# mike-gimelfarb/bboptpy

Hardware: AMD Instinct MI355X
Metric: candidate-evals/sec (higher is better)
Workload: dtype f64; 1 GPU; ActiveCMAES n=128 np=4096 rosenbrock, 256 independent populations per GPU in lockstep; populations_per_gpu=256, n=128, np=4096, objective=rosenbrock

## Files before the change

bboptpy_amd/csrc/bbo_cma.hip:

```cpp
#include "bbo_cma_kernels.hpp"
#include "bbo_sep_kernels.hpp"
#include "bbo_chol_kernels.hpp"
#include "bbo_eig_mw.hpp"

#include <algorithm>
#include <atomic>
#include <cmath>
#include <cstdlib>
#include <limits>

namespace bbo {

namespace {

enum { K_SAMPLE = 0, K_RANK, K_WHITEN, K_GRAM, K_PATHS, K_COV, K_EIGEN, K_POST, K_STOP, K_COUNT };
static const char *const K_NAMES[K_COUNT] = { "bbo:cma_sample_eval", "bbo:cma_rank", "bbo:cma_whiten", "bbo:cma_gram", "bbo:cma_paths", "bbo:cma_cov", "bbo:cma_eigen", "bbo:cma_post", "bbo:cma_history_stop" };

int pick_maxt(int ld)
{
    const int per_wave = ((ld >> 4) + 3) / 4;
    if (per_wave <= 1) return 1;
    if (per_wave <= 2) return 2;
    if (per_wave <= 4) return 4;
    return 8;
// ... 537 lines not shown
        if (c.ld == 128 && (long) c.npop * c.mu_pad >= 256 * 128) {
            const int rw = rows_per_workgroup((long) c.npop * c.mu_pad, 2048);
            add(UK_WHITEN128, K_WHITEN, (c.mu_pad + rw - 1) / rw, c.npop, 1, 512, (size_t) (128 * 128 + 128) * sizeof(double),
                    rw);
        } else
            add(UK_WHITEN, K_WHITEN, c.mu_pad / 16, c.npop, 1, 256, (size_t) (16 * (c.ld + 2) + 64) * sizeof(double),
                    pick_maxt(c.ld));
    }
    if (c.ld != 128)
        add(UK_GRAM, K_GRAM, c.splits, (LT + 4 * GRAM_TPW - 1) / (4 * GRAM_TPW), c.npop, 256, gram_lds_bytes(c.ld, c.rps),
                gram_ldy(c.ld));
    else if (d_.dbg & DBG_GRAM128_LDS)
        add(UK_GRAM128, K_GRAM, c.splits, c.npop, 1, 256, (size_t) (2 * G128_CH * G128_LDY + 4 * G128_CH) * sizeof(double));
    else
        add(UK_GRAM128S, K_GRAM, c.splits, c.npop, 1, 256);
    if (c.lazy_isc && c.n >= 64 && !(d_.dbg & DBG_PATHS_LAZY256))
        add(UK_PATHS_LAZY1K, K_PATHS, c.npop, 1, 1, 1024);
    else
        add(c.lazy_isc ? UK_PATHS_LAZY : UK_PATHS, K_PATHS, c.npop, 1, 1, 256);
    if (with_cov) add(UK_COV, K_COV, (c.n * (c.n + 1) / 2 + 255) / 256, c.npop, 1, 256);
    return r;
}

static auto whiten_kernel(int maxt) -> void (*)(CmaDev, CmaConst)
{
    switch (maxt) {
    case 1: return cma_whiten<1>;
    case 2: return cma_whiten<2>;
    case 4: return cma_whiten<4>;
    default: return cma_whiten<8>;
    }
}

// ... 10 lines not shown
        };
        timed(s.slot, [&] {
            switch (s.k) {
            case UK_CHOL_PATHS: go(chol_paths, 0); break;
            case UK_CHOL_CPRIME: go(chol_cprime, 0); break;
            case UK_CHOL_FACTOR: go(chol_factor, 0, s.arg); break;
            case UK_SEP_MOMENTS: go(sep_moments, 0); break;
            case UK_SEP_PATHS: go(sep_paths, 0); break;
            case UK_WHITEN128: go(cma_whiten128, 132 * 1024, s.arg); break;
            case UK_WHITEN: go(whiten_kernel(s.arg), s.arg == 8 ? 80 * 1024 : 0); break;
            case UK_GRAM128S: go(cma_gram128s, 0); break;
            case UK_GRAM128: go(cma_gram128, 80 * 1024); break;
            case UK_GRAM: go(cma_gram, (int) GRAM_LDS_MAX, s.arg); break;
            case UK_PATHS: go(cma_paths, 0); break;
            case UK_PATHS_LAZY: go(cma_paths_lazy, 0); break;
            case UK_PATHS_LAZY1K: go(cma_paths_lazy1k, 0); break;
            case UK_COV: go(cma_cov, 0); break;
            }
        });
    }
    last_update_ = r;
}

int CmaEngine::next_mw_xcd()
{
    static std::atomic<int> counter { 0 };
    return counter.fetch_add(1) & 7;
}

EigRoute CmaEngine::eig_route(bool spread_ok, bool fuse_ok) const
{
// ... 5 lines not shown
    const EigPlan pl_lds = eig_plan(c.n, c.ld);
    r.split = pl_lds.use_lds && pl_lds.threads == 512 && pl_lds.dc && c.npop <= split_maxp_
            && !(dbg & (DBG_QL | DBG_DC_NO_MERGES | DBG_DC_NO_LEAVES | DBG_TRED_L2 | DBG_EIG_ONE_WG));
    const EigPlan pl = r.split ? eig_plan_split(c.n, c.ld) : pl_lds;
    spread_ok = spread_ok && !mw_disabled_;
    const bool fixed_shape = c.n == 128 && c.ld == 128 && !d_.stamps
            && !(dbg & (DBG_EIG_IN_KERNEL | DBG_EIG_GENERIC128));
    bool big_spread = false, wy4_packs = false, fcols_closed = false;
    if (c.n <= 16 && c.n >= 2 && c.ld == 16 && !(dbg & DBG_NO_EIGEN_SMALL))
        add(EK_EIGEN_SMALL);
    else if (pl.threads < 512)
        add(pl.threads == 128 ? EK_EIGEN_128 : EK_EIGEN_256);
    else if (fixed_shape && c.npop > split_maxp_ && c.lazy_isc) {
        r.fixed = true;
        r.forms_c = fuse_ok && !(dbg & DBG_COV_UNFUSED);
        add(r.forms_c ? EK_EIGEN_FX128 : EK_EIGEN_FX128U);
    } else if (pl.use_lds)
        add(EK_EIGEN);
    else if (pl.hybrid && !(dbg & (DBG_QL | DBG_TRED_L2 | DBG_EIG_ONE_WG))) {
        if (r.split) {
            r.fixed = fixed_shape;
            add(r.fixed ? EK_EIGEN_R1_FX128 : EK_EIGEN_R1);
        } else if (spread_ok && !(dbg & DBG_TRED_ONE_WG)) {
            r.mw_workgroups = (long) c.npop * MW_G;
            const int istop = (dbg & DBG_TRED_ALL_SPREAD) ? 1 : 128;
            add(EK_TRED_MW, istop);
            if (istop > 1) add(EK_TRED_TAIL);
        } else
            add(EK_EIGEN_G1);
        add(EK_EIG_HALVES);
// ... 29 lines not shown
            add(EK_EIG_WY4_512);
        else if ((dbg & DBG_QL) || !pl.hybrid)
            add(EK_EIG_GEMM, 1);
        else if ((long) c.npop * ((c.n + 15) / 16) <= 256 && !(dbg & DBG_WY_PER_WAVE)) {
            wy4_packs = c.lazy_isc != 0;
            add(EK_EIG_WY4, wy4_packs ? (fcols_closed ? 2 : 1) : 0);
        } else
            add(EK_EIG_WY);
    }
    const bool packed_by_eigen = c.lazy_isc && pl.dc && pl.reg_path && !(dbg & DBG_QL);
    r.post = r.step[0].k != EK_EIGEN_SMALL && !packed_by_eigen && !wy4_packs;
    if (r.post) add(c.ld <= 128 ? EK_POST_MFMA : EK_POST);
    return r;
}

void CmaEngine::launch_eigen(EigRoute r)
{
    const CmaConst &c = c_;
    if (r.mw_workgroups && !mw_reserve(r.mw_workgroups)) r = eig_route(false, r.forms_c);
    last_route_ = r;
    if (c.variant >= 2) return;
    const EigPlan pl_lds = eig_plan(c.n, c.ld), pl = r.split ? eig_plan_split(c.n, c.ld) : pl_lds;
    const EigFxArgs fa { d_.C, d_.B, d_.D, d_.BDp, d_.eig_work, d_.scal, c.eigenfreq, c.honor_stop,
            c.splits, c.variant, d_.gram_part, d_.pc, c.cc, c.c1, c.cmu, c.cneg, c.alphaold };
    auto per_matrix = [&](auto kernel, int threads, const EigPlan &p, auto... args) {
        allow_lds((const void*) kernel, 160 * 1024 - 768);
        hipLaunchKernelGGL(kernel, dim3(c.npop), dim3(threads), p.lds_bytes, stream_, args...);
    };
    auto per_columns = [&](auto kernel, int w, int threads, auto... args) {
        hipLaunchKernelGGL(kernel, dim3((c.n + w - 1) / w, c.npop), dim3(threads), 0, stream_, d_, c_, args...);
    };
    timer_.begin(stream_, K_EIGEN);
    for (int i = 0; i < r.count; i++) {
        if (i == r.timed) {
            timer_.end(stream_);
            BBO_HIP(hipGetLastError());
        }
        const int arg = r.step[i].arg;
        switch (r.step[i].k) {
// ... 125 lines not shown
void CmaEngine::generation(bool honor_stop)
{
    if (small_fused_ok()) {
        launch_small(1, honor_stop);
        return;
    }
    small_fused_ = false;
    c_.honor_stop = honor_stop ? 1 : 0;
    launch_sample_eval();
    if (obj_.needs_host()) host_evaluate();
    else if (obj_.is_program()) program_evaluate();
    launch_rank();
    const EigRoute route = eig_route(true, true);
    launch_update(!route.forms_c);
    launch_eigen(route);
    launch_history_stop();
}

void CmaEngine::phase(int which)
{
    BBO_REQUIRE(inited_, "phase before init");
    BBO_HIP(hipSetDevice(params_.device));
    c_.honor_stop = 0;
    d_.mw_fault = mw_fault_from_env();
    switch (which) {
    case BBO_PHASE_SAMPLE_EVALUATE:
        launch_sample_eval();
        if (obj_.needs_host()) host_evaluate();
        else if (obj_.is_program()) program_evaluate();
        break;
    case BBO_PHASE_RANK: launch_rank(); break;
// ... 240 lines not shown
    if (k == "eig_stage") return o.one(s.eig_stage);
    if (k == "eig_mw_fail") return o.one(s.eig_mw_fail);
    if (k == "chol_repairs") {
        if (c.variant != 3) throw Error(BBO_ERR_KEY, "'chol_repairs' belongs to CholeskyCMAES");
        int r = 0;
        chol_repairs_.download(&r, 1, p);
        return o.one(r);
    }
    if (c.variant == 3 && k == "chol_tri") return o.one(chol_tri_ ? 1 : 0);
    if (c.variant == 3 && k == "stol") return o.one(c.stol);
    if (c.variant == 3 && k == "ranked") return o.one(c.ranked);
    if (k == "eig_mw_off") return o.one(mw_disabled_ ? 1 : 0);
    if (k == "eig_split_maxp") return o.one(split_maxp_);
    if (k == "eig_fixed128") return o.one(last_route_.fixed ? 1 : 0);
    if (k == "cov_fused") return o.one(last_route_.forms_c ? 1 : 0);
    if (k == "eig_route") {
        double ids[sizeof(last_route_.step) / sizeof(last_route_.step[0])];
        for (int i = 0; i < last_route_.count; i++) ids[i] = last_route_.step[i].k;
        return o.copy(ids, last_route_.count);
    }
    if (k == "rank_route") return o.one(last_rank_);
    if (k == "sample_route") return o.one(last_sample_.k);
    if (k == "sample_lean") return o.one(last_sample_.full);
    if (k == "sample_transposed") return o.one(last_sample_.transposed);
    if (k == "sample128_rowlayout") return o.one(sample128_rowlayout_ ? 1 : 0);
    if (k == "update_route") {
        double ids[sizeof(last_update_.step) / sizeof(last_update_.step[0])];
        for (int i = 0; i < last_update_.count; i++) ids[i] = last_update_.step[i].k;
        return o.copy(ids, last_update_.count);
    }
// ... 135 lines not shown
        chol_tri_ = in[0] != 0.;
        return 1;
    }
    if (k == "sample_wide_max") {
        sample_wide_max_tiles_ = (long) in[0];
        return 1;
    }
    if (k == "sample128_rowlayout") {
        sample128_rowlayout_ = in[0] != 0.;
        return 1;
    }
    if (k == "sample128_min") {
        sample128_min_rows_ = (long) in[0];
        return 1;
    }
    if (k == "eig_split_maxp") {
        split_maxp_ = (int) in[0];
        return 1;
    }
    if (k == "stop_off") {
        c_.stop_off = (int) in[0];
        return 1;
    }
    if (k == "ftarget") {
        c_.ftarget = in[0];
        return 1;
    }
    if (k == "eig_stamps") {
        if (stamps_.count != 48) stamps_.alloc(48);
        BBO_HIP(hipStreamSynchronize(stream_));
// ... 53 lines not shown
```

bboptpy_amd/csrc/bbo_cma.hpp:

```cpp
#pragma once

#include "bbo_engine.hpp"

namespace bbo {

struct CmaScal {
    double sigma;
    double fbest, fworst;
    double pslen;
    double ybw[4];
    int ibw[4];
    int it, fev;
    int flag;
    int stop;
    int hsig;
    int eigenlastev, eigen_done;
    int hist_head, hist_len;
    int basis_ok;
    int eig_stage;
    int eig_mw_fail;
};

struct CmaConst {
    int n, ld;
// ... 96 lines not shown
    EK_POST, EK_POST_MFMA
};

struct EigRoute {
    struct Step {
        EigKernel k;
        int arg;
    };
    Step step[12];
    int count;
    int timed;
    bool split;
    bool post;
    bool fixed;
    bool forms_c;
    long mw_workgroups;
};

enum SampleKernel : int {
    SK_NONE = -1,
    SK_SEP_16 = 0, SK_SEP_64_512, SK_SEP_64_512_LEAN, SK_SEP_SUM, SK_SEP_SUM4, SK_SEP_64,
    SK_EVAL128, SK_EVAL128_TRI, SK_TILE8, SK_TILE8_TRI,
    SK_EVAL64_1_8, SK_EVAL64_1, SK_EVAL64_2,
    SK_TILE16, SK_EVAL_4, SK_EVAL_8
};

struct SampleRoute {
    SampleKernel k;
    int gx, gy, block;
    size_t lds;
// ... 7 lines not shown
    UK_CHOL_PATHS = 0, UK_CHOL_CPRIME, UK_CHOL_FACTOR, UK_SEP_MOMENTS, UK_SEP_PATHS,
    UK_WHITEN128, UK_WHITEN, UK_GRAM128S, UK_GRAM128, UK_GRAM,
    UK_PATHS, UK_PATHS_LAZY, UK_PATHS_LAZY1K, UK_COV
};

struct UpdateRoute {
    struct Step {
        UpdateKernel k;
        int slot;
        int gx, gy, gz, block;
        size_t lds;
        int arg;
    };
    Step step[4];
    int count;
};

class CmaEngine: public Engine<CmaScal> {
public:
    static constexpr const char *HANDLE_NAME = "not a CMA-ES handle";
    explicit CmaEngine(const bbo_params &p);
    ~CmaEngine() override;

    void init(int n, const double *lower, const double *upper, const double *guess,
            const ObjectiveSpec &obj) override;
    void solution(int population, double *x_out, int *n_evals, int *converged) override;
    void optimize(int n, const double *lower, const double *upper, const double *guess,
            const ObjectiveSpec &obj, double *x_out, int *n_evals, int *converged) override;
    int get(const std::string &key, int population, double *out, int cap) override;
    int set(const std::string &key, int population, const double *in, int count) override;
    int dimension() const override { return c_.n; }
// ... 41 lines not shown

    CmaConst c_ {};
    CmaDev d_ {};
    bool keep_bc_ = false;
    bool basis_maybe_stale_ = false;
    DevBuf<double> mw_buf_;
    unsigned long long mw_launch_ = 0;
    bool mw_disabled_ = false;
    int mw_xcd_ = next_mw_xcd();
    static int next_mw_xcd();
    long sample_wide_max_tiles_ = 512;
    long sample128_min_rows_ = 256 * 128;
    bool chol_tri_ = true;
    bool sample128_rowlayout_ = false;
    int split_maxp_ = 32;
    EigRoute last_route_ {};
    SampleRoute last_sample_ { SK_NONE };
    UpdateRoute last_update_ {};
    bool small_fused_ = false;
    int last_rank_ = -1;
    bool rank_wrote_norms_ = false;
    int last_n_ = -1;

    DevBuf<double> zn2_, csep_, A_;
    DevBuf<double> X_, f_, xmean_, xold_, pc_, ps_, C_, B_, D_, isc_, BDp_, ISp_, S_,
            gram_part_, mean_part_, hist_best_, hist_kth_, eig_work_, weights_, zinject_, zrecord_;
    DevBuf<double> coef_tab_;
    DevBuf<int> rank_, order_, chol_repairs_, coef_stamp_;
    void coef_tab_forget();
    DevBuf<long long> stamps_;
// ... 10 lines not shown
```

bboptpy_amd/csrc/bbo_cma_kernels.hpp:

```cpp
#pragma once

#include "bbo_cma.hpp"
#include "bbo_objectives.hpp"
#include "bbo_rng.hpp"
#include "bbo_eig.hpp"
#include "bbo_rank.hpp"

namespace bbo {

typedef double d4_t __attribute__((ext_vector_type(4)));

#define BBO_INF (__builtin_huge_val())

__device__ inline void cma_draw_quad(const CmaDev &d, const CmaConst &c, int p, int row, int q,
        int gen, uint32_t sw, const double2 *tab, double (&z)[4])
{
    const int j0 = cma_quad_col0(q);
    z[0] = z[1] = z[2] = z[3] = 0.;
    if (row < c.lambda && j0 < c.n) {
        if (d.zinject) {
            const double *zi = d.zinject + ((size_t) p * c.lambda + row) * c.n;
#pragma unroll
            for (int i = 0; i < 4; i++)
                if (j0 + 4 * i < c.n) z[i] = zi[j0 + 4 * i];
// ... 1278 lines not shown
__global__ __launch_bounds__(256, 2) void cma_gram128s(CmaDev d, CmaConst c)
{
    const int p = blockIdx.y, s = blockIdx.x;
    if (pop_frozen(c, d.scal + p)) return;
    __shared__ double coef[4][2 * 2 * G128_CH];
    const int lane = threadIdx.x & 63, wave = threadIdx.x >> 6;
    const bool use_tab = d.coef_tab && !(d.dbg & DBG_GRAM_LOOKUP) && d.coef_stamp[p] == d.scal[p].it + 1;
    switch (wave) {
    case 0: gram128_stream<0>(d, c, p, s, coef[0], lane, use_tab); break;
    case 1: gram128_stream<1>(d, c, p, s, coef[1], lane, use_tab); break;
    case 2: gram128_stream<2>(d, c, p, s, coef[2], lane, use_tab); break;
    default: gram128_stream<3>(d, c, p, s, coef[3], lane, use_tab); break;
    }
}

template<bool LAZY = false, int T = 256>
__device__ __forceinline__ void paths_body(const CmaDev &d, const CmaConst &c, int p)
{
    CmaScal *sc = d.scal + p;
    if (pop_frozen(c, sc)) return;
    __shared__ double dm[512];
    __shared__ double red[T / 64];
    const int tid = threadIdx.x, ld = c.ld;
    double *xmean = d.xmean + (size_t) p * ld, *xold = d.xold + (size_t) p * ld;
    double *ps = d.ps + (size_t) p * ld, *pc = d.pc + (size_t) p * ld;
    const double sigma = sc->sigma;

    for (int j = tid; j < ld; j += T) {
        double sum = 0.;
        {
            const double *mp = d.mean_part + (size_t) p * c.splits * ld + j;
            int s = 0;
            for (; s + 8 <= c.splits; s += 8) {
                double x[8];
#pragma unroll
// ... 3 lines not shown
                for (int u = 0; u < 8; u++) sum += x[u];
            }
            for (; s < c.splits; s++) sum += mp[(size_t) s * ld];
        }
        const double xo = xmean[j];
        sum = xo + sigma * sum;
        double xn = 0.;
        if (j < c.n) {
            xn = c.variant == 1 ? xo * (1. - c.cm) + sum * c.cm : sum;
            if (c.bound) xn = fmax(d.lower[j], fmin(xn, d.upper[j]));
        }
        xold[j] = xo;
        xmean[j] = xn;
        dm[j] = xn - xo;
    }
    __syncthreads();

    const double csc = sqrt(c.cs * (2. - c.cs) * c.mueff);
    const double den = c.variant == 1 ? c.cm * sigma : sigma;
    const double *isc = d.isc + (size_t) p * ld * ld;
    double ssq = 0.;
    if (LAZY && sc->basis_ok) {
        constexpr int HN = T / 128;
        constexpr int RS = T / 16, NU = 128 / RS;
        __shared__ double sv[256], cv[256], part[HN - 1][128];
        const double *B = d.B + (size_t) p * ld * ld, *D = d.D + (size_t) p * ld;
        for (int jb = 0; jb < c.n; jb += 128) {
            const int j = jb + (tid & 127), h = tid >> 7;
            double t0 = 0., t1 = 0., t2 = 0., t3 = 0.;
            if (j < c.n) {
                int i = h;
                for (; i + 7 * HN < c.n; i += 8 * HN) {
                    double b[8];
#pragma unroll
                    for (int u = 0; u < 8; u++) b[u] = B[(size_t) (i + HN * u) * ld + j];
                    t0 += b[0] * dm[i] + b[4] * dm[i + 4 * HN];
                    t1 += b[1] * dm[i + HN] + b[5] * dm[i + 5 * HN];
                    t2 += b[2] * dm[i + 2 * HN] + b[6] * dm[i + 6 * HN];
                    t3 += b[3] * dm[i + 3 * HN] + b[7] * dm[i + 7 * HN];
                }
                for (; i < c.n; i += HN) t0 += B[(size_t) i * ld + j] * dm[i];
            }
            const double t = (t0 + t1) + (t2 + t3);
            if (h > 0) part[h - 1][tid & 127] = t;
            __syncthreads();
            if (h == 0) {
                double tt = t;
#pragma unroll
                for (int q = 0; q < HN - 1; q++) tt += part[q][tid & 127];
                sv[j] = j < c.n ? tt / D[j] : 0.;
            }
            __syncthreads();
        }
        for (int ib = 0; ib < c.n; ib += 128) {
            const int g = tid & 15, r = ib + (tid >> 4);
            double a[NU];
#pragma unroll
            for (int u = 0; u < NU; u++) {
                const int i = r + RS * u;
                double tot = 0.;
                for (int kb = 0; kb < c.n; kb += 128) {
                    double x[8];
#pragma unroll
                    for (int k = 0; k < 8; k++) {
                        const int j = kb + g + 16 * k;
                        x[k] = (i < c.n && j < c.n) ? B[(size_t) i * ld + j] * sv[j] : 0.;
                    }
                    const double part8 = ((x[0] + x[1]) + (x[2] + x[3])) + ((x[4] + x[5]) + (x[6] + x[7]));
                    tot = kb == 0 ? part8 : tot + part8;
                }
                a[u] = tot;
            }
#pragma unroll
            for (int u = 0; u < NU; u++) {
                const double v = group_sum<16>(a[u]);
                if (g == 0 && r + RS * u < c.n) cv[r + RS * u] = v;
            }
        }
        __syncthreads();
        for (int i = tid; i < ld; i += T) {
            const double v = i < c.n ? (1. - c.cs) * ps[i] + csc * cv[i] / den : 0.;
            ps[i] = v;
            ssq += v * v;
        }
    } else {
        for (int i = tid; i < ld; i += T) {
            double v = 0.;
            if (i < c.n) {
                double acc = 0.;
                for (int j = 0; j < c.n; j++) acc += isc[(size_t) j * ld + i] * dm[j];
                v = (1. - c.cs) * ps[i] + csc * acc / den;
            }
            ps[i] = v;
// ... 26 lines not shown
        if (sc->it >= c.hlen && sc->fworst - sc->fbest == 0.) sg *= exp(0.2 + c.cs / c.damps);
        sc->sigma = sg;
        sc->hsig = hsig;
        sc->pslen = pslen;
    }
}

__global__ __launch_bounds__(256) void cma_paths(CmaDev d, CmaConst c)
{
    paths_body<false>(d, c, blockIdx.x);
}
__global__ __launch_bounds__(256) void cma_paths_lazy(CmaDev d, CmaConst c)
{
    paths_body<true>(d, c, blockIdx.x);
}
__global__ __launch_bounds__(1024) void cma_paths_lazy1k(CmaDev d, CmaConst c)
{
    paths_body<true, 1024>(d, c, blockIdx.x);
}

__device__ __forceinline__ void cov_body(const CmaDev &d, const CmaConst &c, int p, int bx)
{
    const CmaScal *sc = d.scal + p;
    if (pop_frozen(c, sc)) return;
    const int q = bx * 256 + threadIdx.x;
    const int total = c.n * (c.n + 1) / 2;
    if (q >= total) return;
    int i, j;
    tri_tile(q, i, j);
    const int ld = c.ld;
    double *C = d.C + (size_t) p * ld * ld;
    const double *pc = d.pc + (size_t) p * ld;
    const double cij = C[(size_t) i * ld + j];
// ... 200 lines not shown
    }
    if (mode == 2) {
        for (int q = q0 + tid; q < q1; q += 256) {
            const int t4 = q >> 6, l = q & 63;
            const int nt = t4 / KS, ks = t4 - nt * KS;
            const int i = nt * 16 + (l & 15), j = 4 * ks + (l >> 4);
            ISp[q] = (i < n && j < n) ? isc[(size_t) i * ld + j] : 0.;
        }
    }
}

__device__ __forceinline__ void history_stop_body(const CmaDev &d, const CmaConst &c, int p, int lane)
{
    CmaScal *sc = d.scal + p;
    if (pop_frozen(c, sc)) return;
    const int ld = c.ld, n = c.n;
    double *hb = d.hist_best + (size_t) p * c.hlen, *hk = d.hist_kth + (size_t) p * c.hlen;
    const double *f = d.f + (size_t) p * c.lambda_pad;
    const int *order = d.order + (size_t) p * c.lambda_pad;
    int it = sc->it;
    int head = sc->hist_head, len = sc->hist_len;
    double fbest = sc->fbest, fworst = sc->fworst;

    if (it < c.mit) {
        head = (head + 1) % c.hlen;
        if (lane == 0) {
            hb[head] = f[order[0]];
            hk[head] = f[order[c.ik]];
        }
        if (len < c.hlen) len++;
        wave_sync();
        if (len == c.hlen) {
            double lo = BBO_INF, hi = -BBO_INF;
            for (int k = lane; k < c.hlen; k += 64) {
                lo = fmin(lo, hb[k]);
                hi = fmax(hi, hb[k]);
            }
#pragma unroll
            for (int off = 32; off > 0; off >>= 1) {
                lo = fmin(lo, __shfl_xor(lo, off, 64));
                hi = fmax(hi, __shfl_xor(hi, off, 64));
            }
            fbest = lo;
            fworst = hi;
        }
    }
    it++;
    wave_sync();

    const double sigma = sc->sigma;
    const double *pc = d.pc + (size_t) p * ld, *xm = d.xmean + (size_t) p * ld;
    const double *C = d.C + (size_t) p * ld * ld, *B = d.B + (size_t) p * ld * ld;
    const double *D = d.D + (size_t) p * ld;
    int flag = 0;
    const int off = c.stop_off;
    if (it >= c.mit) {
        flag = 1;
    } else if (f[order[0]] <= c.ftarget) {
        flag = 10;
    } else if (!(off & 4) && it >= c.hlen && fworst - fbest < c.tol) {
        flag = 2;
    } else {
        if (!(off & 8) && len >= n) {
            int eq = 0;
            for (int i = lane; i < n; i += 64) {
                const int idx = (c.hlen + head - i) % c.hlen;
                eq += hb[idx] == hk[idx];
            }
#pragma unroll
            for (int off = 32; off > 0; off >>= 1) eq += __shfl_xor(eq, off, 64);
            if (3 * eq >= n) flag = 3;
        }
        const bool sep = c.variant == 2;
        if (!flag && !(off & 16)) {
            int bad = 0;
            for (int i = lane; i < n; i += 64) {
                const double sd = sep ? D[i] : sqrt(C[(size_t) i * ld + i]);
                bad |= (fmax(pc[i], sd) * sigma / c.sigma0 >= c.tol);
            }
            if (!__any(bad)) flag = 4;
        }
        if (!flag && !(off & 32) && sigma / c.sigma0 > 1.0e20 * D[n - 1]) flag = 5;
        if (!flag && !(off & 128) && D[n - 1] > 1.0e7 * D[0]) flag = 7;
        if (!flag && !(off & 256)) {
            const int iaxis = n - 1 - ((it - 1) % n);
            int moved = 0;
            if (sep) {
                moved = xm[iaxis] != xm[iaxis] + 0.1 * sigma * D[iaxis];
            } else {
                for (int i = lane; i < n; i += 64)
                    moved |= (xm[i] != xm[i] + 0.1 * sigma * D[iaxis] * B[(size_t) iaxis * ld + i]);
            }
            if (!__any(moved)) flag = 8;
        }
        if (!flag && !(off & 512)) {
            int stuck = 0;
            for (int i = lane; i < n; i += 64) {
                const double sd = sep ? D[i] : sqrt(C[(size_t) i * ld + i]);
                stuck |= (xm[i] == xm[i] + 0.2 * sigma * sd);
            }
            if (__any(stuck)) flag = 9;
        }
    }
    if (lane == 0) {
        sc->it = it;
        sc->hist_head = head;
        sc->hist_len = len;
        sc->fbest = fbest;
        sc->fworst = fworst;
        sc->flag = flag;
        if (flag) sc->stop = 1;
        else if (sc->fev >= c.mfev) sc->stop = 2;
    }
}

__global__ __launch_bounds__(64) void cma_history_stop(CmaDev d, CmaConst c)
{
    history_stop_body(d, c, blockIdx.x, threadIdx.x);
}

constexpr int SMALL_FUSED_MAXP = 512;

__host__ __device__ inline int small_state_doubles(const CmaConst &c)
{
    const int ld = c.ld, ld2 = ld * ld, lp = c.lambda_pad;
    return lp * ld
            + 2 * lp + lp
            + 5 * ld
// ... 228 lines not shown
```

bboptpy_amd/csrc/bbo_eig.hpp:

```cpp
#pragma once

#include <type_traits>

#include "bbo_cma.hpp"
#include "bbo_eig_ql.hpp"
#include "bbo_eig_dc.hpp"

namespace bbo {

typedef double d4_eig __attribute__((ext_vector_type(4)));

constexpr int EIG_THREADS = 512;
constexpr int EIG_NMAX = 512;

struct EigPlan {
    int threads;
    int use_lds;
    int reg_path;
    int dc;
    int hybrid;
    int lda;
    int rc;
    int vl;
    size_t lds_bytes;
// ... 36 lines not shown
        pl.lds_bytes = fixed + mat + (size_t) 2 * pl.rc * 16;
    } else {
        pl.use_lds = 0;
        pl.lda = (n + 31) & ~31;
        if (pl.hybrid) {
            pl.rc = 0;
            pl.lds_bytes = fixed + (size_t) 128 * 130 * sizeof(double);
        } else {
            pl.rc = 2048;
            pl.lds_bytes = fixed + (size_t) 2 * pl.rc * 16;
        }
    }
    return pl;
}

inline EigPlan eig_plan_split(int n, int ld)
{
    EigPlan pl = eig_plan(n, ld);
    pl.threads = EIG_THREADS;
    pl.vl = 128 + 2;
    pl.reg_path = 0;
    pl.hybrid = 1;
    pl.use_lds = 0;
    pl.lda = (n + 31) & ~31;
    pl.rc = 0;
    const size_t ints = (size_t) (2 * EIG_MAXSEQ * 3 + 8) * sizeof(int);
    const size_t vecs = ((size_t) EIG_NVEC * pl.vl + eig_part_doubles(pl.vl, false, true)) * sizeof(double);
    pl.lds_bytes = vecs + ints + (size_t) 128 * 130 * sizeof(double);
    return pl;
}

struct CovCoef {
    double c1, c2, decay;
};
__device__ __forceinline__ CovCoef cov_coef(const CmaConst &c, int hsig)
{
    const double c2 = (1. - hsig) * c.cc * (2. - c.cc);
    const double decay = c.variant == 1 ? (1. - c.c1 - c.cmu + c.cneg * c.alphaold)
                                        : (1. - c.c1 - c.cmu);
    return CovCoef { c.c1, c2, decay };
}
__device__ __forceinline__ double cov_elem(const CovCoef &k, double cij, double pci, double pcj)
{
    return k.decay * cij + k.c1 * (pci * pcj + k.c2 * cij);
}

template<int AMAX>
__device__ inline double tred_matvec(const double (&a_)[4][8], double (&ur)[4][8], const double *uv,
        int q)
{
#pragma unroll
    for (int a = 0; a < AMAX; a++)
#pragma unroll
        for (int b = 0; b < 8; b += 2) {
            const double2 t2 = *reinterpret_cast<const double2*>(&uv[32 * a + 8 * q + b]);
            ur[a][b] = t2.x;
            ur[a][b + 1] = t2.y;
        }
    double acc0 = 0., acc1 = 0.;
// ... 887 lines not shown
            if (ok[u]) {
                As[i * LB + j] = sum;
                As[j * LB + i] = sum;
            }
        }
    }
    __syncthreads();
    for (int q = tid; q < N * (N / 2); q += TT) {
        const int r = q >> 6, c2 = (q & 63) * 2;
        *reinterpret_cast<double2*>(&C[r * N + c2]) = make_double2(As[r * LB + c2], As[r * LB + c2 + 1]);
    }
}

template<int TT, bool LDSM, int HYB = 1, int STAGE = 0, bool FX = false, bool PRO = false>
__device__ __forceinline__ void cma_eigen_impl(const CmaDev &d, const CmaConst &c, const EigPlan &pl,
        int force)
{
    const int p = blockIdx.x;
    CmaScal *sc = d.scal + p;
    if (c.honor_stop && sc->stop != 0) return;
    bool due = true;
    if (STAGE == 2 || STAGE == 4) {
        if (sc->eig_stage != 1) return;
    } else if (STAGE == 3) {
    } else
    if (!force && !((double) (sc->fev - sc->eigenlastev) > c.eigenfreq)) {
        if (threadIdx.x == 0) {
            sc->eigen_done = 0;
            sc->eig_stage = 0;
        }
        if (!PRO) return;
// ... 9 lines not shown
    double *gv = wv + nv;
    double *hvec = gv + nv;
    double *td = hvec + nv;
    double *uh0 = td + nv, *uh1 = uh0 + nv;
    double *part = uh1 + nv - 2;
    double2 *rot = reinterpret_cast<double2*>(part
            + eig_part_doubles(nv, pl.reg_path != 0, pl.hybrid != 0));
    int *ibuf = reinterpret_cast<int*>(rot + 2 * pl.rc);
    int *desc = ibuf;
    int *nseq = ibuf + 2 * EIG_MAXSEQ * 3;
    int *sdone = nseq + 2;
    int *perm = reinterpret_cast<int*>(uv);
    EigMat A { LDSM ? reinterpret_cast<double*>(ibuf + 2 * EIG_MAXSEQ * 3 + 8)
                    : d.eig_work + (size_t) p * 4 * eig_slab(ld), pl.lda };
    double *C = d.C + (size_t) p * ld * ld;

#define EIG_STAMP(slot) do { if (d.stamps && p == 0 && tid == 0) d.stamps[slot] = wall_clock64(); } while (0)
    EIG_STAMP(0);
    if (tid < 2) {
        dv[-1 - tid] = 0.;
        ev[-1 - tid] = 0.;
    }
    double *tri = d.eig_work + (size_t) (4 * p + 3) * eig_slab(ld);
    if (STAGE == 3) {
        if (tri[4 * n + 1] != (force ? 2. : 1.) || sc->eig_mw_fail) return;
        constexpr int LB = 130;
        EigMat Ast { reinterpret_cast<double*>(ibuf + 2 * EIG_MAXSEQ * 3 + 8), LB };
        const double *L11 = d.eig_work + (size_t) (4 * p) * eig_slab(ld);
        for (int q = tid; q < 128 * 64; q += T) {
            const int r = q >> 6, c2 = (q & 63) * 2;
// ... 12 lines not shown
        for (int r = wave; r < 128; r += T / 64)
            for (int cidx = lane; cidx < n; cidx += 64) Vout[(size_t) r * n + cidx] = cidx < r ? Ast(r, cidx) : 0.;
        if (tid == 0) sc->eig_stage = 1;
        return;
    }
    if (STAGE == 2 || STAGE == 4) {
        for (int i = tid; i < n; i += T) {
            dv[i] = STAGE == 2 ? tri[3 * n + i] : tri[i];
            ev[i] = tri[n + i];
            hvec[i] = tri[2 * n + i];
        }
        __syncthreads();
    } else {
    if (PRO) {
        eig_cov_prologue128<TT>(d, c, sc, p, A.a, tid);
        if (!due) return;
        eig_tred_accum_reg128<TT>(A.a, A.ld, n, A, dv, ev, uv, wv, gv, hvec, td, tid, nullptr, A.a, A.ld, true,
                !(pl.dc && !(d.dbg & DBG_QL)));
    } else if (LDSM) {
        eig_tred_accum_reg128<TT>(C, ld, n, A, dv, ev, uv, wv, gv, hvec, td, tid,
                (d.stamps && p == 0) ? d.stamps : nullptr, A.a, A.ld, true,
                !(pl.dc && !(d.dbg & DBG_QL)));
    } else if (TT == EIG_THREADS && !LDSM) {
        const bool hybrid = HYB != 0;
        EigMat Ast { reinterpret_cast<double*>(ibuf + 2 * EIG_MAXSEQ * 3 + 8), 128 };
        if (hybrid && !(d.dbg & DBG_QL) && !(d.dbg & DBG_TRED_L2))
            eig_tred_sym256(C, ld, n, A, dv, ev, uv, wv, gv, hvec, td, nv, tid,
                    (d.stamps && p == 0) ? d.stamps : nullptr, Ast, false,
                    d.eig_work + (size_t) (4 * p + 1) * eig_slab(ld));
        else
        eig_tred_accum_global(C, ld, n, A, dv, ev, uv, wv, gv, hvec, td, part, nv, tid,
// ... 94 lines not shown
            const double dk = dc_key(dv[k]);
            r += (dk < kj) || (dk == kj && k < j);
        }
        perm[j] = r;
        gv[r] = dj;
    }
    }
    __syncthreads();
    const double lo = gv[0], hi = gv[n - 1];
    __syncthreads();
    if (lo <= 0.) {
        const double shift = fmax(hi, 0.) / 1e14;
        for (int i = tid; i < n; i += T) {
            gv[i] = fmax(gv[i], 0.) + shift;
            C[(size_t) i * ld + i] += shift;
        }
        __syncthreads();
    }
    const double lo2 = gv[0], hi2 = gv[n - 1];
    __syncthreads();
    if (hi2 > 1e14 * lo2) {
        const double shift = hi2 / 1e14 - lo2;
        for (int i = tid; i < n; i += T) {
            gv[i] += shift;
            C[(size_t) i * ld + i] += shift;
        }
        __syncthreads();
    }
    double *Dp = d.D + (size_t) p * ld;
    double *Bp = d.B + (size_t) p * ld * ld;
    for (int i = tid; i < ld; i += T) Dp[i] = i < n ? sqrt(gv[i]) : 1.;
    if (!use_dc)
        for (int k = wave; k < n; k += T / 64)
            for (int j = lane; j < n; j += 64) Bp[(size_t) k * ld + perm[j]] = A(k, j);
    if (tid == 0) {
        sc->eigenlastev = sc->fev;
        sc->eigen_done = 1;
        sc->eig_stage = 0;
    }
    if (use_dc && LDSM && c.lazy_isc) {
        __syncthreads();
        for (int j = tid; j < n; j += T) dv[j] = sqrt(gv[j]);
        __syncthreads();
        double *BDp = d.BDp + (size_t) p * ld * ld;
        const int KS = ld >> 2;
        for (int q = tid; q < ld * ld; q += T) {
            const int t4 = q >> 6, l = q & 63;
            const int nt = t4 / KS, ks = t4 - nt * KS;
            const int i = nt * 16 + (l & 15), j = 4 * ks + (l >> 4);
            BDp[q] = (i < n && j < n) ? A(i, j) * dv[j] : 0.;
        }
        if (tid == 0) sc->basis_ok = 1;
    }
    EIG_STAMP(5);
#undef EIG_STAMP
}

__global__ __launch_bounds__(512) void cma_eigen(CmaDev d, CmaConst c, EigPlan pl, int force)
{
    cma_eigen_impl<512, true>(d, c, pl, force);
}
__global__ __launch_bounds__(512) void cma_eigen_g(CmaDev d, CmaConst c, EigPlan pl, int force)
{
    cma_eigen_impl<512, false, 1>(d, c, pl, force);
}
__global__ __launch_bounds__(512) void cma_eigen_b(CmaDev d, CmaConst c, EigPlan pl, int force)
{
    cma_eigen_impl<512, false, 0>(d, c, pl, force);
}
struct EigFxArgs {
    double *C, *B, *D, *BDp, *eig_work;
    CmaScal *scal;
    double eigenfreq;
    int honor_stop;
    int splits, variant;
    const double *gram_part, *pc;
    double cc, c1, cmu, cneg, alphaold;
};
__device__ __forceinline__ void eig_fx_cov_args(const EigFxArgs &a, CmaDev &d, CmaConst &c)
{
    d.gram_part = const_cast<double*>(a.gram_part);
    d.pc = const_cast<double*>(a.pc);
    c.splits = a.splits;
    c.variant = a.variant;
    c.cc = a.cc;
    c.c1 = a.c1;
    c.cmu = a.cmu;
    c.cneg = a.cneg;
    c.alphaold = a.alphaold;
}
constexpr EigPlan EIG_FX_PLAN = eig_plan(128, 128);
template<bool PRO>
// ... 2 lines not shown
    static_assert(EIG_FX_PLAN.use_lds == 1 && EIG_FX_PLAN.dc == 1 && EIG_FX_PLAN.reg_path == 1
            && EIG_FX_PLAN.threads == 512 && EIG_FX_PLAN.vl == 130, "cma_eigen_fx128: the plan of n = 128");
    CmaDev d {};
    d.C = a.C;
    d.B = a.B;
    d.D = a.D;
    d.BDp = a.BDp;
    d.eig_work = a.eig_work;
    d.scal = a.scal;
    CmaConst c {};
    c.n = c.ld = 128;
    c.lazy_isc = 1;
    c.honor_stop = a.honor_stop;
    c.eigenfreq = a.eigenfreq;
    if (PRO) eig_fx_cov_args(a, d, c);
    cma_eigen_impl<512, true, 1, 0, true, PRO>(d, c, EIG_FX_PLAN, 0);
}
__global__ __launch_bounds__(512) void cma_eigen_fx128(EigFxArgs a)
{
    cma_eigen_fx128_body<true>(a);
}
__global__ __launch_bounds__(512) void cma_eigen_fx128u(EigFxArgs a)
{
    cma_eigen_fx128_body<false>(a);
}
__global__ __launch_bounds__(512) void cma_eigen_r1_fx128(EigFxArgs a)
{
    CmaDev d {};
    d.C = a.C;
    d.eig_work = a.eig_work;
    d.scal = a.scal;
// ... 767 lines not shown
```

Baseline: 737.2 million candidate-evals/s.

## Fold history/stop check into fixed-128 eigen kernel and stage B in LDS for paths

Moves the per-population history and stop-criteria check into the fused fixed-shape n=128 eigen kernel, so the separate history_stop launch is skipped on that route. The stop logic is factored into a shared core, reads the diagonal of C from a saved LDS copy, and takes its constants from a small device buffer that is uploaded only when they change. Separately, the 1024-thread lazy paths kernel now stages the 128x128 basis B into padded LDS before the two matrix-vector products instead of reading it from global memory twice. This adds LDS pressure, a possible host sync when the constants change, and more code in an already large eigen kernel.

```diff
diff --git a/bboptpy_amd/csrc/bbo_cma.hip b/bboptpy_amd/csrc/bbo_cma.hip
--- a/bboptpy_amd/csrc/bbo_cma.hip
+++ b/bboptpy_amd/csrc/bbo_cma.hip
@@ -575,9 +575,10 @@
         add(UK_GRAM128, K_GRAM, c.splits, c.npop, 1, 256, (size_t) (2 * G128_CH * G128_LDY + 4 * G128_CH) * sizeof(double));
     else
         add(UK_GRAM128S, K_GRAM, c.splits, c.npop, 1, 256);
-    if (c.lazy_isc && c.n >= 64 && !(d_.dbg & DBG_PATHS_LAZY256))
-        add(UK_PATHS_LAZY1K, K_PATHS, c.npop, 1, 1, 1024);
-    else
+    if (c.lazy_isc && c.n >= 64 && !(d_.dbg & DBG_PATHS_LAZY256)) {
+        r.paths_lds = paths_lds_ && c.ld == 128;
+        add(UK_PATHS_LAZY1K, K_PATHS, c.npop, 1, 1, 1024, r.paths_lds ? PATHS_LDS_BYTES : 0, r.paths_lds ? 1 : 0);
+    } else
         add(c.lazy_isc ? UK_PATHS_LAZY : UK_PATHS, K_PATHS, c.npop, 1, 1, 256);
     if (with_cov) add(UK_COV, K_COV, (c.n * (c.n + 1) / 2 + 255) / 256, c.npop, 1, 256);
     return r;
@@ -618,7 +619,7 @@
             case UK_GRAM: go(cma_gram, (int) GRAM_LDS_MAX, s.arg); break;
             case UK_PATHS: go(cma_paths, 0); break;
             case UK_PATHS_LAZY: go(cma_paths_lazy, 0); break;
-            case UK_PATHS_LAZY1K: go(cma_paths_lazy1k, 0); break;
+            case UK_PATHS_LAZY1K: go(cma_paths_lazy1k, s.arg ? (int) PATHS_LDS_BYTES : 0, s.arg); break;
             case UK_COV: go(cma_cov, 0); break;
             }
         });
@@ -654,6 +655,7 @@
     else if (fixed_shape && c.npop > split_maxp_ && c.lazy_isc) {
         r.fixed = true;
         r.forms_c = fuse_ok && !(dbg & DBG_COV_UNFUSED);
+        r.folds_stop = r.forms_c && stop_fold_;
         add(r.forms_c ? EK_EIGEN_FX128 : EK_EIGEN_FX128U);
     } else if (pl.use_lds)
         add(EK_EIGEN);
@@ -713,6 +715,23 @@
     return r;
 }
 
+const StopConst *CmaEngine::stop_const_sync()
+{
+    StopConst k;
+    std::memset(&k, 0, sizeof(k));
+    k = stop_const(d_, c_);
+    if (stopk_.count != sizeof(k)) {
+        stopk_.alloc(sizeof(k));
+        stopk_host_.clear();
+    }
+    if (stopk_host_.size() != sizeof(k) || std::memcmp(stopk_host_.data(), &k, sizeof(k)) != 0) {
+        stopk_host_.assign(reinterpret_cast<const unsigned char*>(&k), reinterpret_cast<const unsigned char*>(&k) + sizeof(k));
+        BBO_HIP(hipStreamSynchronize(stream_));
+        stopk_.upload(stopk_host_.data(), sizeof(k));
+    }
+    return reinterpret_cast<const StopConst*>(stopk_.p);
+}
+
 void CmaEngine::launch_eigen(EigRoute r)
 {
     const CmaConst &c = c_;
@@ -721,7 +740,8 @@
     if (c.variant >= 2) return;
     const EigPlan pl_lds = eig_plan(c.n, c.ld), pl = r.split ? eig_plan_split(c.n, c.ld) : pl_lds;
     const EigFxArgs fa { d_.C, d_.B, d_.D, d_.BDp, d_.eig_work, d_.scal, c.eigenfreq, c.honor_stop,
-            c.splits, c.variant, d_.gram_part, d_.pc, c.cc, c.c1, c.cmu, c.cneg, c.alphaold };
+            c.splits, c.variant, d_.gram_part, d_.pc, c.cc, c.c1, c.cmu, c.cneg, c.alphaold,
+            r.folds_stop ? stop_const_sync() : nullptr };
     auto per_matrix = [&](auto kernel, int threads, const EigPlan &p, auto... args) {
         allow_lds((const void*) kernel, 160 * 1024 - 768);
         hipLaunchKernelGGL(kernel, dim3(c.npop), dim3(threads), p.lds_bytes, stream_, args...);
@@ -877,7 +897,7 @@
     const EigRoute route = eig_route(true, true);
     launch_update(!route.forms_c);
     launch_eigen(route);
-    launch_history_stop();
+    if (!last_route_.folds_stop) launch_history_stop();
 }
 
 void CmaEngine::phase(int which)
@@ -1148,6 +1168,10 @@
     if (k == "eig_split_maxp") return o.one(split_maxp_);
     if (k == "eig_fixed128") return o.one(last_route_.fixed ? 1 : 0);
     if (k == "cov_fused") return o.one(last_route_.forms_c ? 1 : 0);
+    if (k == "stop_folded") return o.one(last_route_.folds_stop ? 1 : 0);
+    if (k == "stop_fold") return o.one(stop_fold_ ? 1 : 0);
+    if (k == "paths_lds") return o.one(paths_lds_ ? 1 : 0);
+    if (k == "paths_lds_used") return o.one(last_update_.paths_lds ? 1 : 0);
     if (k == "eig_route") {
         double ids[sizeof(last_route_.step) / sizeof(last_route_.step[0])];
         for (int i = 0; i < last_route_.count; i++) ids[i] = last_route_.step[i].k;
@@ -1313,6 +1337,14 @@
         sample128_min_rows_ = (long) in[0];
         return 1;
     }
+    if (k == "stop_fold") {
+        stop_fold_ = in[0] != 0.;
+        return 1;
+    }
+    if (k == "paths_lds") {
+        paths_lds_ = in[0] != 0.;
+        return 1;
+    }
     if (k == "eig_split_maxp") {
         split_maxp_ = (int) in[0];
         return 1;
diff --git a/bboptpy_amd/csrc/bbo_cma.hpp b/bboptpy_amd/csrc/bbo_cma.hpp
--- a/bboptpy_amd/csrc/bbo_cma.hpp
+++ b/bboptpy_amd/csrc/bbo_cma.hpp
@@ -134,6 +134,7 @@
     bool post;
     bool fixed;
     bool forms_c;
+    bool folds_stop;
     long mw_workgroups;
 };
 
@@ -171,7 +172,10 @@
     };
     Step step[4];
     int count;
-};
+    bool paths_lds;
+};
+
+struct StopConst;
 
 class CmaEngine: public Engine<CmaScal> {
 public:
@@ -243,6 +247,11 @@
     bool chol_tri_ = true;
     bool sample128_rowlayout_ = false;
     int split_maxp_ = 32;
+    bool stop_fold_ = true;
+    bool paths_lds_ = true;
+    DevBuf<unsigned char> stopk_;
+    std::vector<unsigned char> stopk_host_;
+    const StopConst *stop_const_sync();
     EigRoute last_route_ {};
     SampleRoute last_sample_ { SK_NONE };
     UpdateRoute last_update_ {};
diff --git a/bboptpy_amd/csrc/bbo_cma_kernels.hpp b/bboptpy_amd/csrc/bbo_cma_kernels.hpp
--- a/bboptpy_amd/csrc/bbo_cma_kernels.hpp
+++ b/bboptpy_amd/csrc/bbo_cma_kernels.hpp
@@ -1316,11 +1316,84 @@
     }
 }
 
+template<int T>
+__device__ __forceinline__ void paths_lazy_products(const CmaConst &c, const double *B, const int ldb,
+        const double *D, const double *dm, double *sv, double *cv, double (*part)[128])
+{
+    const int tid = threadIdx.x;
+    constexpr int HN = T / 128;
+    constexpr int RS = T / 16, NU = 128 / RS;
+    for (int jb = 0; jb < c.n; jb += 128) {
+        const int j = jb + (tid & 127), h = tid >> 7;
+        double t0 = 0., t1 = 0., t2 = 0., t3 = 0.;
+        if (j < c.n) {
+            int i = h;
+            for (; i + 7 * HN < c.n; i += 8 * HN) {
+                double b[8];
+#pragma unroll
+                for (int u = 0; u < 8; u++) b[u] = B[(size_t) (i + HN * u) * ldb + j];
+                t0 += b[0] * dm[i] + b[4] * dm[i + 4 * HN];
+                t1 += b[1] * dm[i + HN] + b[5] * dm[i + 5 * HN];
+                t2 += b[2] * dm[i + 2 * HN] + b[6] * dm[i + 6 * HN];
+                t3 += b[3] * dm[i + 3 * HN] + b[7] * dm[i + 7 * HN];
+            }
+            for (; i < c.n; i += HN) t0 += B[(size_t) i * ldb + j] * dm[i];
+        }
+        const double t = (t0 + t1) + (t2 + t3);
+        if (h > 0) part[h - 1][tid & 127] = t;
+        __syncthreads();
+        if (h == 0) {
+            double tt = t;
+#pragma unroll
+            for (int q = 0; q < HN - 1; q++) tt += part[q][tid & 127];
+            sv[j] = j < c.n ? tt / D[j] : 0.;
+        }
+        __syncthreads();
+    }
+    for (int ib = 0; ib < c.n; ib += 128) {
+        const int g = tid & 15, r = ib + (tid >> 4);
+        double a[NU];
+#pragma unroll
+        for (int u = 0; u < NU; u++) {
+            const int i = r + RS * u;
+            double tot = 0.;
+            for (int kb = 0; kb < c.n; kb += 128) {
+                double x[8];
+#pragma unroll
+                for (int k = 0; k < 8; k++) {
+                    const int j = kb + g + 16 * k;
+                    x[k] = (i < c.n && j < c.n) ? B[(size_t) i * ldb + j] * sv[j] : 0.;
+                }
+                const double part8 = ((x[0] + x[1]) + (x[2] + x[3])) + ((x[4] + x[5]) + (x[6] + x[7]));
+                tot = kb == 0 ? part8 : tot + part8;
+            }
+            a[u] = tot;
+        }
+#pragma unroll
+        for (int u = 0; u < NU; u++) {
+            const double v = group_sum<16>(a[u]);
+            if (g == 0 && r + RS * u < c.n) cv[r + RS * u] = v;
+        }
+    }
+}
+
+constexpr int PATHS_LDS_LD = 144;
+typedef double paths_d2 __attribute__((ext_vector_type(2)));
+constexpr size_t PATHS_LDS_BYTES = (size_t) 128 * PATHS_LDS_LD * sizeof(double);
+
 template<bool LAZY = false, int T = 256>
-__device__ __forceinline__ void paths_body(const CmaDev &d, const CmaConst &c, int p)
+__device__ __forceinline__ void paths_body(const CmaDev &d, const CmaConst &c, int p, int b_lds = 0)
 {
     CmaScal *sc = d.scal + p;
     if (pop_frozen(c, sc)) return;
+    extern __shared__ __attribute__((aligned(16))) double paths_bs[];
+    const bool copy_b = LAZY && T == 1024 && b_lds && sc->basis_ok;
+    paths_d2 bq[8] = {};
+    if (T == 1024 && copy_b) {
+        const paths_d2 *Bg = reinterpret_cast<const paths_d2*>(d.B + (size_t) p * 128 * 128);
+#pragma unroll
+        for (int u = 0; u < 8; u++) bq[u] = Bg[threadIdx.x + 1024 * u];
+    }
     __shared__ double dm[512];
     __shared__ double red[T / 64];
     const int tid = threadIdx.x, ld = c.ld;
@@ -1354,6 +1427,11 @@
         xmean[j] = xn;
         dm[j] = xn - xo;
     }
+    if (T == 1024 && copy_b) {
+#pragma unroll
+        for (int u = 0; u < 8; u++)
+            *reinterpret_cast<paths_d2*>(&paths_bs[((tid >> 6) + 16 * u) * PATHS_LDS_LD + 2 * (tid & 63)]) = bq[u];
+    }
     __syncthreads();
 
     const double csc = sqrt(c.cs * (2. - c.cs) * c.mueff);
@@ -1362,61 +1440,11 @@
     double ssq = 0.;
     if (LAZY && sc->basis_ok) {
         constexpr int HN = T / 128;
-        constexpr int RS = T / 16, NU = 128 / RS;
         __shared__ double sv[256], cv[256], part[HN - 1][128];
-        const double *B = d.B + (size_t) p * ld * ld, *D = d.D + (size_t) p * ld;
-        for (int jb = 0; jb < c.n; jb += 128) {
-            const int j = jb + (tid & 127), h = tid >> 7;
-            double t0 = 0., t1 = 0., t2 = 0., t3 = 0.;
-            if (j < c.n) {
-                int i = h;
-                for (; i + 7 * HN < c.n; i += 8 * HN) {
-                    double b[8];
-#pragma unroll
-                    for (int u = 0; u < 8; u++) b[u] = B[(size_t) (i + HN * u) * ld + j];
-                    t0 += b[0] * dm[i] + b[4] * dm[i + 4 * HN];
-                    t1 += b[1] * dm[i + HN] + b[5] * dm[i + 5 * HN];
-                    t2 += b[2] * dm[i + 2 * HN] + b[6] * dm[i + 6 * HN];
-                    t3 += b[3] * dm[i + 3 * HN] + b[7] * dm[i + 7 * HN];
-                }
-                for (; i < c.n; i += HN) t0 += B[(size_t) i * ld + j] * dm[i];
-            }
-            const double t = (t0 + t1) + (t2 + t3);
-            if (h > 0) part[h - 1][tid & 127] = t;
-            __syncthreads();
-            if (h == 0) {
-                double tt = t;
-#pragma unroll
-                for (int q = 0; q < HN - 1; q++) tt += part[q][tid & 127];
-                sv[j] = j < c.n ? tt / D[j] : 0.;
-            }
-            __syncthreads();
-        }
-        for (int ib = 0; ib < c.n; ib += 128) {
-            const int g = tid & 15, r = ib + (tid >> 4);
-            double a[NU];
-#pragma unroll
-            for (int u = 0; u < NU; u++) {
-                const int i = r + RS * u;
-                double tot = 0.;
-                for (int kb = 0; kb < c.n; kb += 128) {
-                    double x[8];
-#pragma unroll
-                    for (int k = 0; k < 8; k++) {
-                        const int j = kb + g + 16 * k;
-                        x[k] = (i < c.n && j < c.n) ? B[(size_t) i * ld + j] * sv[j] : 0.;
-                    }
-                    const double part8 = ((x[0] + x[1]) + (x[2] + x[3])) + ((x[4] + x[5]) + (x[6] + x[7]));
-                    tot = kb == 0 ? part8 : tot + part8;
-                }
-                a[u] = tot;
-            }
-#pragma unroll
-            for (int u = 0; u < NU; u++) {
-                const double v = group_sum<16>(a[u]);
-                if (g == 0 && r + RS * u < c.n) cv[r + RS * u] = v;
-            }
-        }
+        if (T == 1024 && copy_b)
+            paths_lazy_products<T>(c, paths_bs, PATHS_LDS_LD, d.D + (size_t) p * ld, dm, sv, cv, part);
+        else
+            paths_lazy_products<T>(c, d.B + (size_t) p * ld * ld, ld, d.D + (size_t) p * ld, dm, sv, cv, part);
         __syncthreads();
         for (int i = tid; i < ld; i += T) {
             const double v = i < c.n ? (1. - c.cs) * ps[i] + csc * cv[i] / den : 0.;
@@ -1473,9 +1501,9 @@
 {
     paths_body<true>(d, c, blockIdx.x);
 }
-__global__ __launch_bounds__(1024) void cma_paths_lazy1k(CmaDev d, CmaConst c)
-{
-    paths_body<true, 1024>(d, c, blockIdx.x);
+__global__ __launch_bounds__(1024) void cma_paths_lazy1k(CmaDev d, CmaConst c, int b_lds)
+{
+    paths_body<true, 1024>(d, c, blockIdx.x, b_lds);
 }
 
 __device__ __forceinline__ void cov_body(const CmaDev &d, const CmaConst &c, int p, int bx)
@@ -1706,104 +1734,9 @@
 {
     CmaScal *sc = d.scal + p;
     if (pop_frozen(c, sc)) return;
-    const int ld = c.ld, n = c.n;
-    double *hb = d.hist_best + (size_t) p * c.hlen, *hk = d.hist_kth + (size_t) p * c.hlen;
-    const double *f = d.f + (size_t) p * c.lambda_pad;
-    const int *order = d.order + (size_t) p * c.lambda_pad;
-    int it = sc->it;
-    int head = sc->hist_head, len = sc->hist_len;
-    double fbest = sc->fbest, fworst = sc->fworst;
-
-    if (it < c.mit) {
-        head = (head + 1) % c.hlen;
-        if (lane == 0) {
-            hb[head] = f[order[0]];
-            hk[head] = f[order[c.ik]];
-        }
-        if (len < c.hlen) len++;
-        wave_sync();
-        if (len == c.hlen) {
-            double lo = BBO_INF, hi = -BBO_INF;
-            for (int k = lane; k < c.hlen; k += 64) {
-                lo = fmin(lo, hb[k]);
-                hi = fmax(hi, hb[k]);
-            }
-#pragma unroll
-            for (int off = 32; off > 0; off >>= 1) {
-                lo = fmin(lo, __shfl_xor(lo, off, 64));
-                hi = fmax(hi, __shfl_xor(hi, off, 64));
-            }
-            fbest = lo;
-            fworst = hi;
-        }
-    }
-    it++;
-    wave_sync();
-
-    const double sigma = sc->sigma;
-    const double *pc = d.pc + (size_t) p * ld, *xm = d.xmean + (size_t) p * ld;
-    const double *C = d.C + (size_t) p * ld * ld, *B = d.B + (size_t) p * ld * ld;
-    const double *D = d.D + (size_t) p * ld;
-    int flag = 0;
-    const int off = c.stop_off;
-    if (it >= c.mit) {
-        flag = 1;
-    } else if (f[order[0]] <= c.ftarget) {
-        flag = 10;
-    } else if (!(off & 4) && it >= c.hlen && fworst - fbest < c.tol) {
-        flag = 2;
-    } else {
-        if (!(off & 8) && len >= n) {
-            int eq = 0;
-            for (int i = lane; i < n; i += 64) {
-                const int idx = (c.hlen + head - i) % c.hlen;
-                eq += hb[idx] == hk[idx];
-            }
-#pragma unroll
-            for (int off = 32; off > 0; off >>= 1) eq += __shfl_xor(eq, off, 64);
-            if (3 * eq >= n) flag = 3;
-        }
-        const bool sep = c.variant == 2;
-        if (!flag && !(off & 16)) {
-            int bad = 0;
-            for (int i = lane; i < n; i += 64) {
-                const double sd = sep ? D[i] : sqrt(C[(size_t) i * ld + i]);
-                bad |= (fmax(pc[i], sd) * sigma / c.sigma0 >= c.tol);
-            }
-            if (!__any(bad)) flag = 4;
-        }
-        if (!flag && !(off & 32) && sigma / c.sigma0 > 1.0e20 * D[n - 1]) flag = 5;
-        if (!flag && !(off & 128) && D[n - 1] > 1.0e7 * D[0]) flag = 7;
-        if (!flag && !(off & 256)) {
-            const int iaxis = n - 1 - ((it - 1) % n);
-            int moved = 0;
-            if (sep) {
-                moved = xm[iaxis] != xm[iaxis] + 0.1 * sigma * D[iaxis];
-            } else {
-                for (int i = lane; i < n; i += 64)
-                    moved |= (xm[i] != xm[i] + 0.1 * sigma * D[iaxis] * B[(size_t) iaxis * ld + i]);
-            }
-            if (!__any(moved)) flag = 8;
-        }
-        if (!flag && !(off & 512)) {
-            int stuck = 0;
-            for (int i = lane; i < n; i += 64) {
-                const double sd = sep ? D[i] : sqrt(C[(size_t) i * ld + i]);
-                stuck |= (xm[i] == xm[i] + 0.2 * sigma * sd);
-            }
-            if (__any(stuck)) flag = 9;
-        }
-    }
-    if (lane == 0) {
-        sc->it = it;
-        sc->hist_head = head;
-        sc->hist_len = len;
-        sc->fbest = fbest;
-        sc->fworst = fworst;
-        sc->flag = flag;
-        if (flag) sc->stop = 1;
-        else if (sc->fev >= c.mfev) sc->stop = 2;
-    }
+    const size_t ld = c.ld;
+    history_stop_core(stop_const(d, c), sc, p, lane, d.D + p * ld, d.B + p * ld * ld, c.ld,
+            d.C + p * ld * ld, c.ld + 1);
 }
 
 __global__ __launch_bounds__(64) void cma_history_stop(CmaDev d, CmaConst c)
diff --git a/bboptpy_amd/csrc/bbo_eig.hpp b/bboptpy_amd/csrc/bbo_eig.hpp
--- a/bboptpy_amd/csrc/bbo_eig.hpp
+++ b/bboptpy_amd/csrc/bbo_eig.hpp
@@ -74,6 +74,8 @@
     return pl;
 }
 
+constexpr int EIG_FX_RC = eig_plan(128, 128).rc;
+
 inline EigPlan eig_plan_split(int n, int ld)
 {
     EigPlan pl = eig_plan(n, ld);
@@ -103,6 +105,120 @@
 __device__ __forceinline__ double cov_elem(const CovCoef &k, double cij, double pci, double pcj)
 {
     return k.decay * cij + k.c1 * (pci * pcj + k.c2 * cij);
+}
+
+struct StopConst {
+    double *hist_best, *hist_kth;
+    const double *f;
+    const int *order;
+    const double *xmean, *pc;
+    double tol, sigma0, ftarget;
+    int n, ld, lambda_pad, hlen, ik, mit, mfev, variant, stop_off;
+};
+__host__ __device__ inline StopConst stop_const(const CmaDev &d, const CmaConst &c)
+{
+    return StopConst { d.hist_best, d.hist_kth, d.f, d.order, d.xmean, d.pc, c.tol, c.sigma0, c.ftarget,
+            c.n, c.ld, c.lambda_pad, c.hlen, c.ik, c.mit, c.mfev, c.variant, c.stop_off };
+}
+__device__ __forceinline__ void history_stop_core(const StopConst &c, CmaScal *sc, int p, int lane,
+        const double *D, const double *B, int ldb, const double *Cd, int ldc)
+{
+    const int ld = c.ld, n = c.n;
+    double *hb = c.hist_best + (size_t) p * c.hlen, *hk = c.hist_kth + (size_t) p * c.hlen;
+    const double *f = c.f + (size_t) p * c.lambda_pad;
+    const int *order = c.order + (size_t) p * c.lambda_pad;
+    int it = sc->it;
+    int head = sc->hist_head, len = sc->hist_len;
+    double fbest = sc->fbest, fworst = sc->fworst;
+
+    if (it < c.mit) {
+        head = (head + 1) % c.hlen;
+        if (lane == 0) {
+            hb[head] = f[order[0]];
+            hk[head] = f[order[c.ik]];
+        }
+        if (len < c.hlen) len++;
+        wave_sync();
+        if (len == c.hlen) {
+            double lo = __builtin_huge_val(), hi = -__builtin_huge_val();
+            for (int k = lane; k < c.hlen; k += 64) {
+                lo = fmin(lo, hb[k]);
+                hi = fmax(hi, hb[k]);
+            }
+#pragma unroll
+            for (int off = 32; off > 0; off >>= 1) {
+                lo = fmin(lo, __shfl_xor(lo, off, 64));
+                hi = fmax(hi, __shfl_xor(hi, off, 64));
+            }
+            fbest = lo;
+            fworst = hi;
+        }
+    }
+    it++;
+    wave_sync();
+
+    const double sigma = sc->sigma;
+    const double *pc = c.pc + (size_t) p * ld, *xm = c.xmean + (size_t) p * ld;
+    int flag = 0;
+    const int off = c.stop_off;
+    if (it >= c.mit) {
+        flag = 1;
+    } else if (f[order[0]] <= c.ftarget) {
+        flag = 10;
+    } else if (!(off & 4) && it >= c.hlen && fworst - fbest < c.tol) {
+        flag = 2;
+    } else {
+        if (!(off & 8) && len >= n) {
+            int eq = 0;
+            for (int i = lane; i < n; i += 64) {
+                const int idx = (c.hlen + head - i) % c.hlen;
+                eq += hb[idx] == hk[idx];
+            }
+#pragma unroll
+            for (int off = 32; off > 0; off >>= 1) eq += __shfl_xor(eq, off, 64);
+            if (3 * eq >= n) flag = 3;
+        }
+        const bool sep = c.variant == 2;
+        if (!flag && !(off & 16)) {
+            int bad = 0;
+            for (int i = lane; i < n; i += 64) {
+                const double sd = sep ? D[i] : sqrt(Cd[(size_t) i * ldc]);
+                bad |= (fmax(pc[i], sd) * sigma / c.sigma0 >= c.tol);
+            }
+            if (!__any(bad)) flag = 4;
+        }
+        if (!flag && !(off & 32) && sigma / c.sigma0 > 1.0e20 * D[n - 1]) flag = 5;
+        if (!flag && !(off & 128) && D[n - 1] > 1.0e7 * D[0]) flag = 7;
+        if (!flag && !(off & 256)) {
+            const int iaxis = n - 1 - ((it - 1) % n);
+            int moved = 0;
+            if (sep) {
+                moved = xm[iaxis] != xm[iaxis] + 0.1 * sigma * D[iaxis];
+            } else {
+                for (int i = lane; i < n; i += 64)
+                    moved |= (xm[i] != xm[i] + 0.1 * sigma * D[iaxis] * B[(size_t) iaxis * ldb + i]);
+            }
+            if (!__any(moved)) flag = 8;
+        }
+        if (!flag && !(off & 512)) {
+            int stuck = 0;
+            for (int i = lane; i < n; i += 64) {
+                const double sd = sep ? D[i] : sqrt(Cd[(size_t) i * ldc]);
+                stuck |= (xm[i] == xm[i] + 0.2 * sigma * sd);
+            }
+            if (__any(stuck)) flag = 9;
+        }
+    }
+    if (lane == 0) {
+        sc->it = it;
+        sc->hist_head = head;
+        sc->hist_len = len;
+        sc->fbest = fbest;
+        sc->fworst = fworst;
+        sc->flag = flag;
+        if (flag) sc->stop = 1;
+        else if (sc->fev >= c.mfev) sc->stop = 2;
+    }
 }
 
 template<int AMAX>
@@ -1020,7 +1136,7 @@
 
 template<int TT, bool LDSM, int HYB = 1, int STAGE = 0, bool FX = false, bool PRO = false>
 __device__ __forceinline__ void cma_eigen_impl(const CmaDev &d, const CmaConst &c, const EigPlan &pl,
-        int force)
+        int force, const StopConst *stopk = nullptr)
 {
     const int p = blockIdx.x;
     CmaScal *sc = d.scal + p;
@@ -1060,6 +1176,8 @@
     EigMat A { LDSM ? reinterpret_cast<double*>(ibuf + 2 * EIG_MAXSEQ * 3 + 8)
                     : d.eig_work + (size_t) p * 4 * eig_slab(ld), pl.lda };
     double *C = d.C + (size_t) p * ld * ld;
+    double *cdiag = PRO ? reinterpret_cast<double*>(rot + 2 * pl.rc) - 128 : nullptr;
+    static_assert(!PRO || (7 * 130 - 2 + 4 * EIG_FX_RC - 128 >= 2200), "cdiag lies in the merge work area");
 
 #define EIG_STAMP(slot) do { if (d.stamps && p == 0 && tid == 0) d.stamps[slot] = wall_clock64(); } while (0)
     EIG_STAMP(0);
@@ -1102,7 +1220,13 @@
     } else {
     if (PRO) {
         eig_cov_prologue128<TT>(d, c, sc, p, A.a, tid);
-        if (!due) return;
+        if (!due) {
+            if (stopk && wave == 0)
+                history_stop_core(*stopk, sc, p, lane, d.D + (size_t) p * ld, d.B + (size_t) p * ld * ld, ld,
+                        A.a, A.ld + 1);
+            return;
+        }
+        if (tid < 128) cdiag[tid] = A.a[tid * A.ld + tid];
         eig_tred_accum_reg128<TT>(A.a, A.ld, n, A, dv, ev, uv, wv, gv, hvec, td, tid, nullptr, A.a, A.ld, true,
                 !(pl.dc && !(d.dbg & DBG_QL)));
     } else if (LDSM) {
@@ -1227,6 +1351,7 @@
         for (int i = tid; i < n; i += T) {
             gv[i] = fmax(gv[i], 0.) + shift;
             C[(size_t) i * ld + i] += shift;
+            if (PRO) cdiag[i] += shift;
         }
         __syncthreads();
     }
@@ -1237,6 +1362,7 @@
         for (int i = tid; i < n; i += T) {
             gv[i] += shift;
             C[(size_t) i * ld + i] += shift;
+            if (PRO) cdiag[i] += shift;
         }
         __syncthreads();
     }
@@ -1264,6 +1390,10 @@
             BDp[q] = (i < n && j < n) ? A(i, j) * dv[j] : 0.;
         }
         if (tid == 0) sc->basis_ok = 1;
+        if (PRO && stopk) {
+            __syncthreads();
+            if (wave == 0) history_stop_core(*stopk, sc, p, lane, dv, A.a, A.ld, cdiag, 1);
+        }
     }
     EIG_STAMP(5);
 #undef EIG_STAMP
@@ -1289,6 +1419,7 @@
     int splits, variant;
     const double *gram_part, *pc;
     double cc, c1, cmu, cneg, alphaold;
+    const StopConst *stopk;
 };
 __device__ __forceinline__ void eig_fx_cov_args(const EigFxArgs &a, CmaDev &d, CmaConst &c)
 {
@@ -1321,7 +1452,7 @@
     c.honor_stop = a.honor_stop;
     c.eigenfreq = a.eigenfreq;
     if (PRO) eig_fx_cov_args(a, d, c);
-    cma_eigen_impl<512, true, 1, 0, true, PRO>(d, c, EIG_FX_PLAN, 0);
+    cma_eigen_impl<512, true, 1, 0, true, PRO>(d, c, EIG_FX_PLAN, 0, PRO ? a.stopk : nullptr);
 }
 __global__ __launch_bounds__(512) void cma_eigen_fx128(EigFxArgs a)
 {
```

New measurement: 740.8 million candidate-evals/s, median of 6. No clear change (+0.5%).
